# facebookresearch/DetectAndTrack

Measured on AMD Instinct MI355X. Metric: clips/sec (8-frame 800px), higher is better.
Workload: dtype bf16; 1 GPU; 3D R-18 FPN3D keypoint R-CNN inference, 4 clip(s) of 1x3x8x768x1344 per step (= per forward) per GPU (kT=3 body+FPN, slice-center 2D heads, per clip: 1000 proposals, 100 detections -> kps_score -> decoded keypoints); mode=infer, weights=random-init (synthetic_params, seed 3), images_per_forward=4, forwards_in_flight=3, clips_in_flight=12, keyframe_dce=False, hip_graph=True, resident_input=True, parallelism=clip-sharded x1 (no data-path collective)

## Files before the change

detectandtrack_amd/core/clip_graph.py:

```python
import numpy as np
import torch

from detectandtrack_amd import workspace as wsmod
from detectandtrack_amd.core import test as engine


def ops_ws_generation():
    from detectandtrack_amd.ops import hip_ops as ops
    return ops.ws_info()[2]


class ClipGraph(object):

    def __init__(self, model, ws, data_like, im_info, im_shape, stream=None, warmup=2, static_data=None, trunk=None):
        self.trunk = trunk
        assert engine.device_results_supported(), 'graph capture needs the device-side post-processing (cfg.HIP.DEVICE_BOX_RESULTS)'
        self.model, self.ws = model, ws
        B = int(trunk[3]) if trunk is not None else int(data_like.shape[0])
        self.scales = [float(v) for v in np.asarray(im_info, dtype=np.float64).reshape(-1, 3)[:, 2]]
        self.im_info = np.asarray(im_info, dtype=np.float32).reshape(-1, 3)
        assert self.im_info.shape[0] == B, 'im_info has %d rows for a blob of %d images' % (self.im_info.shape[0], B)
        self.im_shapes = [tuple(im_shape)] * B if not isinstance(im_shape[0], (tuple, list)) else [tuple(sh) for sh in im_shape]
        assert len(self.im_shapes) == B
        self.stream = stream or torch.cuda.current_stream()
# ... 7 lines not shown
        ws.FeedBlob('im_info', self.im_info)
        with torch.cuda.stream(self.stream):
            for _ in range(warmup):
                self._enqueue()
        torch.cuda.synchronize()
        self.graph = torch.cuda.CUDAGraph()
        with torch.cuda.graph(self.graph, stream=self.stream, capture_error_mode='thread_local'):
            self.dev = self._enqueue()
        torch.cuda.synchronize()
        self.blobs = dict(ws.blobs)
        with torch.cuda.stream(self.stream):
            self.ws_generation = ops_ws_generation()

    def _enqueue(self):
        prev, wsmod._GLOBAL = wsmod._GLOBAL, self.ws
        try:
            if self.trunk is not None:
                self.ws.trunk_ready = self.trunk
            else:
                self.ws.FeedBlob('data', self.static_data)
            self.ws.RunNet(self.model.net.name)
            return engine.enqueue_results_on_device(self.model, self.im_shapes, list(self.scales))
        finally:
            wsmod._GLOBAL = prev

    def launch(self, data_dev, im_info=None, im_shape=None):
        if self.trunk is not None:
            with torch.cuda.stream(self.stream):
                self.graph.replay()
            return self.dev
        assert tuple(data_dev.shape) == tuple(self.static_data.shape), \
            'graph captured for a %s blob, launched with %s' % (tuple(self.static_data.shape), tuple(data_dev.shape))
        if im_info is not None:
            assert np.array_equal(np.asarray(im_info, np.float32).reshape(-1, 3), self.im_info), \
                'graph captured for im_info %s, launched with %s' % (self.im_info.tolist(), np.asarray(im_info).tolist())
        if im_shape is not None:
            shapes = [tuple(im_shape)] * len(self.im_shapes) if not isinstance(im_shape[0], (tuple, list)) else [tuple(sh) for sh in im_shape]
            assert [sh[:2] for sh in shapes] == [sh[:2] for sh in self.im_shapes], (shapes, self.im_shapes)
        with torch.cuda.stream(self.stream):
# ... 17 lines not shown
```

detectandtrack_amd/core/config.py:

```python
import copy
import os
import os.path as osp
from ast import literal_eval

import numpy as np
import yaml

from detectandtrack_amd.utils.collections import AttrDict

_DEFAULTS_YAML = r"""
TRAIN:
  WEIGHTS: ''
  DATASET: ''
  SCALES: [600]
  MAX_SIZE: 1000
  IMS_PER_BATCH: 2
  BATCH_SIZE_PER_IM: 64
  FG_FRACTION: 0.25
  FG_THRESH: 0.5
  BG_THRESH_HI: 0.5
  BG_THRESH_LO: 0.0
  USE_FLIPPED: true
  BBOX_REG: true
  BBOX_THRESH: 0.5
# ... 187 lines not shown


def _to_attr(d, key=None):
    if isinstance(d, dict):
        return AttrDict({k: _to_attr(v, k) for k, v in d.items()})
    if isinstance(d, list) and key in _TUPLE_KEYS:
        return tuple(d)
    return d


def _build_defaults():
    c = _to_attr(yaml.safe_load(_DEFAULTS_YAML))
    c.BBOX_XFORM_CLIP = np.log(1000. / 16.)
    c.PIXEL_MEANS = np.array([[[102.9801, 115.9465, 122.7717]]])
    c.ROOT_DIR = os.getcwd()
    c.HIP = AttrDict({'DTYPE': 'bf16', 'KEYFRAME_DCE': False, 'DEVICE_KPS_DECODE': True, 'FRAME_TRUNK_CACHE': 0,
                      'DEVICE_BOX_RESULTS': True, 'FUSE_STEM_POOL': True, 'RCCL_DIRECT': False,
                      'PIPELINE_DEPTH': 4, 'CLIP_GRAPH': True, 'IMS_PER_FORWARD': 1, 'FUSE_RELU_BWD': True, 'FUSE_RELU_SUM_BWD': True, 'PERSISTENT_CU_SHARE': 50, 'DET_SPARE_ROWS': 4,
                      'DEFER_WGRAD_FINISH': True, 'MAX_GRAPHS_PER_SLOT': 6, 'PAD_TAIL_FORWARD': True,
                      'OVERLAP_ALLREDUCE': True, 'WGRAD_PW_BATCH': 16, 'DEVICE_ROI_SAMPLING': True, 'DECONV_GROUP_IGNORED': False, 'STEM_FROM_UINT8': True,
                      'TRAIN_GROUPED_CONV': False, 'USE_GN': False, 'GN_NUM_GROUPS': 32, 'GN_EPSILON': 1e-5, 'GN_KPS_HEAD': False,
                      'TUBE_SOFT_NMS': False, 'TRACK_CNN_WEIGHTS': '',
                      'TUBE_NMS_OKS': False, 'NMS_OKS_THRESH': 0.3,
                      'NONLOCAL': '', 'NONLOCAL_MAXPOOL': True, 'NONLOCAL_SCALE': True})
    return c


__C = _build_defaults()
cfg = __C
cfg_default = copy.deepcopy(__C)


def reset_cfg():
    fresh = copy.deepcopy(cfg_default)
    for k in list(__C.keys()):
        del __C[k]
    for k, v in fresh.items():
        __C[k] = v

# ... 91 lines not shown
```

detectandtrack_amd/core/pipeline.py:

```python
import collections
import os
import time

import numpy as np
import torch

from detectandtrack_amd.core.config import cfg
from detectandtrack_amd.core import test as engine
from detectandtrack_amd import workspace as wsmod


def _cu_masked_stream(spec):
    import ctypes
    bits = 0
    for part in spec.split('+'):
        lo, hi = [int(v) for v in part.split('-')]
        for b in range(lo, hi + 1):
            bits |= 1 << b
    words = (ctypes.c_uint32 * 8)(*[(bits >> (32 * i)) & 0xffffffff for i in range(8)])
    hip = ctypes.CDLL('libamdhip64.so')
    st = ctypes.c_void_p()
    rc = hip.hipExtStreamCreateWithCUMask(ctypes.byref(st), 8, words)
    assert rc == 0, 'hipExtStreamCreateWithCUMask failed: %d' % rc
    return torch.cuda.ExternalStream(st.value)
# ... 192 lines not shown
            g = s.graphs.get(key)
            if g is None:
                from detectandtrack_amd.core.clip_graph import ClipGraph
                while len(s.graphs) >= self.max_graphs:
                    _, old = s.graphs.popitem(last=False)
                    del old
                    self.graphs_evicted += 1
                g = s.graphs[key] = ClipGraph(self.model, s.ws, data_dev, im_info, im_shapes, stream=s.stream,
                                              static_data=data_dev if in_place else None, trunk=trunk)
                self.graphs_captured += 1
            else:
                s.graphs.move_to_end(key)
            return g.launch(data_dev, im_info=im_info, im_shape=im_shapes), g
        with torch.cuda.stream(s.stream):
            prev, wsmod._GLOBAL = wsmod._GLOBAL, s.ws
            try:
                if trunk is not None:
                    s.ws.trunk_ready = trunk
                else:
                    s.ws.FeedBlob('data', data_dev)
                s.ws.FeedBlob('im_info', np.asarray(im_info, np.float32))
                s.ws.RunNet(self.model.net.name)
                scales = [float(v) for v in np.asarray(im_info, np.float64).reshape(-1, 3)[:, 2]]
                return engine.enqueue_results_on_device(self.model, list(im_shapes), scales), None
            finally:
                wsmod._GLOBAL = prev

    def submit(self, data_dev, im_info, im_shape, tag=None, resident=False):
        slot = self._acquire()
        t0 = time.perf_counter()
        B = int(data_dev.shape[0])
        im_info = np.asarray(im_info, np.float64).reshape(-1, 3)
        assert im_info.shape[0] == B, (im_info.shape, B)
        shapes = [tuple(im_shape)] * B if not isinstance(im_shape[0], (tuple, list)) else [tuple(sh) for sh in im_shape]
        dev, g = self._enqueue(slot, data_dev, im_info, shapes, in_place=False, resident=resident and self.use_graph)
        self.slots[slot].event.record(self.slots[slot].stream)
        self.host_enqueue_s += time.perf_counter() - t0
        self.pending.append((slot, tag, im_info, shapes, dev, None, g))

    def _submit_frames_cached(self, clips, tag, frame_ids):
        from detectandtrack_amd.ops import hip_ops as ops
# ... 154 lines not shown
```

detectandtrack_amd/core/test.py:

```python
from collections import defaultdict

import numpy as np

from detectandtrack_amd.core.config import cfg
from detectandtrack_amd.core.nms_wrapper import nms, soft_nms
from detectandtrack_amd.ops.hip_ops import SOFT_NMS_MAX_BOXES
from detectandtrack_amd.ops.hip_ops import OKS_NMS_MAX_ROWS
from detectandtrack_amd.utils.timer import Timer
from detectandtrack_amd import workspace
import detectandtrack_amd.utils.blob as blob_utils
import detectandtrack_amd.utils.boxes as box_utils
import detectandtrack_amd.utils.keypoints as keypoint_utils


def _get_image_blob(im, num_frames=None):
    per_frame, scales = [], []
    for frame in im:
        ims, sc = blob_utils.prep_im_for_blob(frame, cfg.PIXEL_MEANS, cfg.TEST.SCALES, cfg.TEST.MAX_SIZE)
        per_frame.append(ims)
        scales.append(sc)
    for s in scales:
        assert scales[0] == s
    processed = [frames[i] for i in range(len(per_frame[0])) for frames in per_frame]
    return blob_utils.im_list_to_blob(processed, num_frames), np.array(scales[0])
# ... 169 lines not shown
def _nms_oks_on_device():
    return bool((not _tube_detections() or cfg.HIP.TUBE_NMS_OKS) and cfg.MODEL.NUM_CLASSES == 2 and cfg.KRCNN.NUM_KEYPOINTS == 17 and
                _device_out_cap() <= OKS_NMS_MAX_ROWS)


def device_results_supported():
    return bool(cfg.HIP.DEVICE_BOX_RESULTS and cfg.MODEL.FASTER_RCNN and cfg.TEST.BBOX_REG and
                not ((cfg.TEST.SOFT_NMS.ENABLED or cfg.TEST.BBOX_VOTE.ENABLED) and _tube_detections() and not cfg.HIP.TUBE_SOFT_NMS) and
                not (cfg.TEST.SOFT_NMS.ENABLED and cfg.TEST.RPN_POST_NMS_TOP_N > _soft_nms_capacity()) and
                not cfg.TEST.SVM and not (cfg.KRCNN.NMS_OKS and cfg.MODEL.KEYPOINTS_ON and not _nms_oks_on_device()) and
                (cfg.HIP.DEVICE_KPS_DECODE or not cfg.MODEL.KEYPOINTS_ON))


def rerun_rows_supported(need):
    return not (cfg.KRCNN.NMS_OKS and cfg.MODEL.KEYPOINTS_ON) or int(need) <= OKS_NMS_MAX_ROWS


def enqueue_results_on_device(model, im_shape, im_scale, out_cap=None, image=None):
    from detectandtrack_amd.ops import hip_ops as ops
    ws = workspace.GlobalWorkspace()
    rois = ws.blobs['rois']
    assert rois.kind == 'rois' and rois.count is not None, 'device post-processing expects the on-device proposal blob'
    ni = int(rois.count.numel())
    prob = workspace.blob_as_matrix(ws.blobs['cls_prob'])
    pred = workspace.blob_as_matrix(ws.blobs['bbox_pred'])
    rois_t, rois_n = rois.t if rois.t.dim() == 2 else rois.t.view(-1, rois.t.shape[-1]), rois.count
    if image is not None:
        seg = int(rois_t.shape[0]) // ni
        lo = int(image) * seg
        rois_t, rois_n = rois_t[lo:lo + seg], rois.count.view(-1)[int(image):int(image) + 1]
# ... 7 lines not shown
    dets, kp_rois, n_out = ops.box_results(
        rois_t, rois_n, prob, pred, cfg.MODEL.NUM_CLASSES, T, im_scale, im_shape, cfg.MODEL.BBOX_REG_WEIGHTS,
        float(np.float32(cfg.BBOX_XFORM_CLIP)), cfg.TEST.SCORE_THRESH, cfg.TEST.NMS, D, out_cap,
        cls_agnostic=cfg.MODEL.CLS_AGNOSTIC_BBOX_REG, n_images=ni,
        soft_nms=dict(method=cfg.TEST.SOFT_NMS.METHOD, sigma=cfg.TEST.SOFT_NMS.SIGMA, score_thresh=0.0001)
        if cfg.TEST.SOFT_NMS.ENABLED else None,
        bbox_vote=cfg.TEST.BBOX_VOTE.VOTE_TH if cfg.TEST.BBOX_VOTE.ENABLED else None,
        tubes=bool(cfg.HIP.TUBE_SOFT_NMS))
    xy = None
    if cfg.MODEL.KEYPOINTS_ON:
        if image is not None:
            kp_rois[:, 0] = float(image)
        b = workspace.Blob(kp_rois, 'mat')
        b.count = n_out[0:1] if ni == 1 else n_out[:, 0]
        ws.blobs['keypoint_rois'] = b
        workspace.RunNet(model.keypoint_net.Proto().name)
        heat = ws.blobs['kps_score'].t
        assert heat.shape[1] == cfg.KRCNN.NUM_KEYPOINTS * T, 'Heatmaps must be 17xT'
        xy = ops.heatmaps_to_keypoints(heat.contiguous(), dets, T, cfg.KRCNN.NUM_KEYPOINTS,
                                       cfg.KRCNN.INFERENCE_MIN_SIZE)
        if cfg.KRCNN.NMS_OKS:
            keypoint_utils.check_nms_oks_config()
            dets, xy, _, n_keep = ops.oks_nms(xy, dets, b.count, ni, T, cfg.KRCNN.NUM_KEYPOINTS, cfg.HIP.NMS_OKS_THRESH)
            return dets, n_out, xy, n_keep
    return dets, n_out, xy


def _split_results(d, keyps, num_classes):
    cls_boxes = [[] for _ in range(num_classes)]
    cls_keyps = [[] for _ in range(num_classes)] if keyps is not None else None
    for j in range(1, num_classes):
        sel = np.where(d[:, -1] == j)[0]
        cls_boxes[j] = d[sel, :-1]
        if keyps is not None and j == keypoint_utils.get_person_class_index():
            cls_keyps[j] = [keyps[i] for i in sel]
# ... 130 lines not shown
```

detectandtrack_amd/csrc/elementwise.hip:

```cpp
#include <algorithm>
#include <stdlib.h>

#include "dat_common.h"

namespace {

constexpr int TPB = 256;
inline int grid_for(size_t n, int per_thread = 1) {
    size_t b = (n + (size_t)TPB * per_thread - 1) / ((size_t)TPB * per_thread);
    const size_t cap = 256 * 16;
    return (int)(b < 1 ? 1 : (b > cap ? cap : b));
}

__global__ void zero_even_kernel(float* x, long long n) {
    const long long half = (n + 1) / 2;
    for (long long i = blockIdx.x * (long long)blockDim.x + threadIdx.x; i < half; i += (long long)gridDim.x * blockDim.x)
        x[2 * i] = 0.f;
}

template <bool HAS_BIAS>
__global__ void affine_nd_kernel(const float* __restrict__ x, const float* __restrict__ scale,
                                 const float* __restrict__ bias, float* __restrict__ y, int C, long long inner,
                                 long long total) {
    if ((inner & 3) == 0) {
// ... 177 lines not shown
                if (x >= L) continue;
                const int kx = ox + pad - up * x;
                const float fx = 1.f - fabsf((float)kx - center) / factor;
                const size_t fr = (size_t)r * Tr + t;
                const float v = ElemOf<DT>::ld(sub, ((fr * S + (y >> 1)) * S + (x >> 1)) * cs + ((y & 1) * 2 + (x & 1)) * K + k);
                acc += v * (fy * fx);
            }
        }
        out[i] = acc;
    }
}

template <int DT>
__global__ void kps_finalize_tile_kernel(const void* __restrict__ sub, int S, int cs, int K, int up, float* __restrict__ out) {
    extern __shared__ float low[];
    const int L = 2 * S, M = L * up;
    const int ksz = 2 * up, pad = up / 2;
    const float factor = (float)((ksz + 1) / 2);
    const float center = (ksz % 2 == 1) ? factor - 1.f : factor - 0.5f;
    const int fr = blockIdx.x / K, k = blockIdx.x - fr * K;
    for (int i = threadIdx.x; i < S * S * 4; i += blockDim.x) {
        const int cell = i >> 2, ab = i & 3;
        const int ys = cell / S, xs = cell - ys * S;
        low[(2 * ys + (ab >> 1)) * L + 2 * xs + (ab & 1)] = ElemOf<DT>::ld(sub, ((size_t)fr * S * S + cell) * cs + ab * K + k);
    }
    __syncthreads();
    const int ox = threadIdx.x % M, og = threadIdx.x / M, ng = blockDim.x / M;
    const int x_hi = (ox + pad) / up;
    float* const obase = out + (size_t)blockIdx.x * M * M;
    if (up == 2) {
        const int xa = x_hi, xb = x_hi - 1;
        const bool vxa = xa < L, vxb = xb >= 0;
        const float fxa = 1.f - fabsf((float)(ox + pad - up * xa) - center) / factor;
        const float fxb = 1.f - fabsf((float)(ox + pad - up * xb) - center) / factor;
        for (int oy = og; oy < M; oy += ng) {
            const int ya = (oy + pad) / up, yb = ya - 1;
            const float fya = 1.f - fabsf((float)(oy + pad - up * ya) - center) / factor;
            const float fyb = 1.f - fabsf((float)(oy + pad - up * yb) - center) / factor;
            float acc = 0.f;
            if (ya < L) {
                if (vxa) acc += low[ya * L + xa] * (fya * fxa);
                if (vxb) acc += low[ya * L + xb] * (fya * fxb);
            }
            if (yb >= 0) {
                if (vxa) acc += low[yb * L + xa] * (fyb * fxa);
                if (vxb) acc += low[yb * L + xb] * (fyb * fxb);
            }
            obase[(size_t)oy * M + ox] = acc;
        }
        return;
    }
    for (int oy = og; oy < M; oy += ng) {
        const int y_hi = (oy + pad) / up;
        float acc = 0.f;
        for (int y = y_hi; y >= 0 && oy + pad - up * y < ksz; --y) {
            if (y >= L) continue;
            const int ky = oy + pad - up * y;
            const float fy = 1.f - fabsf((float)ky - center) / factor;
            for (int x = x_hi; x >= 0 && ox + pad - up * x < ksz; --x) {
                if (x >= L) continue;
                const int kx = ox + pad - up * x;
                const float fx = 1.f - fabsf((float)kx - center) / factor;
                acc += low[y * L + x] * (fy * fx);
            }
        }
        obase[(size_t)oy * M + ox] = acc;
    }
}

}

#define DISPATCH_DT(dtype, KERNEL, grid, block, st, ...)                                                  \
    do {                                                                                                  \
        if ((dtype) == DAT_BF16)                                                                          \
            hipLaunchKernelGGL((KERNEL<DAT_BF16>), grid, block, 0, st, __VA_ARGS__);                      \
        else                                                                                              \
            hipLaunchKernelGGL((KERNEL<DAT_F32>), grid, block, 0, st, __VA_ARGS__);                       \
    } while (0)

__global__ void split_bf16x2_kernel(const float* __restrict__ x, uint4* __restrict__ y, long long n8, int c8) {
    for (long long i = blockIdx.x * (long long)blockDim.x + threadIdx.x; i < n8; i += (long long)gridDim.x * blockDim.x) {
        const long long pos = i / c8;
// ... 186 lines not shown
```

detectandtrack_amd/csrc/keypoints.hip:

```cpp
#include "dat_common.h"

namespace {

struct KpParams {
    const float* maps;
    const float* boxes;
    float* out;
    int R, T, K, M, min_size;
    int box_ld;
};

__device__ __forceinline__ void cubic(float t, float c[4]) {
    const float a = -0.75f;
    c[0] = ((a * (t + 1.f) - 5.f * a) * (t + 1.f) + 8.f * a) * (t + 1.f) - 4.f * a;
    c[1] = ((a + 2.f) * t - (a + 3.f)) * t * t + 1.f;
    c[2] = ((a + 2.f) * (1.f - t) - (a + 3.f)) * (1.f - t) * (1.f - t) + 1.f;
    c[3] = 1.0f - c[0] - c[1] - c[2];
}

__device__ __forceinline__ void resample(int src_len, int dst_len, int d, int& i0, float& frac) {
    const double step = 1.0 / ((double)dst_len / (double)src_len);
    const float f = (float)(((double)d + 0.5) * step - 0.5);
    const float fl = floorf(f);
    i0 = (int)fl;
// ... 66 lines not shown
        const int pos = red_i[0];
        const int x_int = pos % mw, y_int = (pos - x_int) / mw;
        const float w_corr = width / (float)mw, h_corr = height / (float)mh;
        const int TK = p.T * p.K, col = t * p.K + k;
        float* o = p.out + (size_t)r * 4 * TK;
        o[0 * TK + col] = (float)(((double)x_int + 0.5) * (double)w_corr + (double)off_x);
        o[1 * TK + col] = (float)(((double)y_int + 0.5) * (double)h_corr + (double)off_y);
        o[2 * TK + col] = red_v[0];
        o[3 * TK + col] = 1.f / red_s[0];
    }
}

constexpr int KD_STRIP = 64;
constexpr int KD_HP = KD_STRIP + 4;

__global__ __launch_bounds__(256) void kps_decode_sep_kernel(const KpParams p) {
    extern __shared__ __attribute__((aligned(16))) float smem_kd[];
    __shared__ float red_v[256];
    __shared__ int red_i[256];
    __shared__ float red_m[256], red_s[256];
    const int tid = threadIdx.x;
    const int k = blockIdx.x % p.K;
    const int t = (blockIdx.x / p.K) % p.T;
    const int r = blockIdx.x / (p.K * p.T);
    const int M = p.M;
    float* map = smem_kd;
    float* Hs = map + ((M * M + 3) & ~3);
    const float* src = p.maps + ((size_t)r * p.T * p.K + (size_t)t * p.K + k) * M * M;
    for (int i = tid; i < M * M; i += 256) map[i] = src[i];

    const float* b = p.boxes + (size_t)r * p.box_ld + t * 4;
    const float off_x = b[0], off_y = b[1];
    const float width = fmaxf(b[2] - b[0], 1.f), height = fmaxf(b[3] - b[1], 1.f);
    int mw = (int)ceilf(width), mh = (int)ceilf(height);
    if (p.min_size > 0) { mw = max(mw, p.min_size); mh = max(mh, p.min_size); }
    const double step_x = 1.0 / ((double)mw / (double)M), step_y = 1.0 / ((double)mh / (double)M);

    float best = -INFINITY;
    int best_i = 0x7fffffff;
    float run_m = -INFINITY, run_s = 0.f;
    const int hx = tid & 63, hr = tid >> 6;
    const int rl = tid >> 2, q = tid & 3;
    for (int x_base = 0; x_base < mw; x_base += KD_STRIP) {
        const int ncol = min(KD_STRIP, mw - x_base);
// ... 70 lines not shown
            red_m[tid] = mm; red_s[tid] = s;
        }
        __syncthreads();
    }
    if (tid == 0) {
        const int pos = red_i[0];
        const int x_int = pos % mw, y_int = (pos - x_int) / mw;
        const float w_corr = width / (float)mw, h_corr = height / (float)mh;
        const int TK = p.T * p.K, col = t * p.K + k;
        float* o = p.out + (size_t)r * 4 * TK;
        o[0 * TK + col] = (float)(((double)x_int + 0.5) * (double)w_corr + (double)off_x);
        o[1 * TK + col] = (float)(((double)y_int + 0.5) * (double)h_corr + (double)off_y);
        o[2 * TK + col] = red_v[0];
        o[3 * TK + col] = 1.f / red_s[0];
    }
}

}

extern "C" int dat_heatmaps_to_keypoints_ld(dat_ctx* ctx, dat_stream s, const float* maps, const float* boxes, int box_ld, int R, int T,
                                            int K, int M, int min_size, float* out);

extern "C" int dat_heatmaps_to_keypoints(dat_ctx* ctx, dat_stream s, const float* maps, const float* boxes, int R, int T,
                                         int K, int M, int min_size, float* out) {
    return dat_heatmaps_to_keypoints_ld(ctx, s, maps, boxes, 4 * T, R, T, K, M, min_size, out);
}

extern "C" int dat_heatmaps_to_keypoints_ld(dat_ctx* ctx, dat_stream s, const float* maps, const float* boxes, int box_ld, int R, int T,
                                            int K, int M, int min_size, float* out) {
    DAT_ENFORCE(ctx, maps && boxes && out && box_ld >= 4 * T, "heatmaps_to_keypoints: null argument / box row stride %d < 4 T", box_ld);
    DAT_ENFORCE(ctx, T >= 1 && K >= 1 && M >= 2 && (size_t)M * M * 4 <= 64 * 1024, "heatmaps_to_keypoints: T %d K %d M %d unsupported", T, K, M);
    if (R == 0) return DAT_OK;
    KpParams p;
    p.maps = maps; p.boxes = boxes; p.out = out; p.R = R; p.T = T; p.K = K; p.M = M; p.min_size = min_size; p.box_ld = box_ld;
    const size_t lds_sep = ((((size_t)M * M + 3) & ~(size_t)3) + (size_t)M * KD_HP) * 4;
    bool sep = ctx->dbg_kps_sep && lds_sep + 4096 <= 160 * 1024;
    if (sep && lds_sep + 4096 > 64 * 1024 && dat_ensure_lds(ctx, (const void*)kps_decode_sep_kernel, 160 * 1024) != DAT_OK) sep = false;
    if (sep) {
        hipLaunchKernelGGL(kps_decode_sep_kernel, dim3((unsigned)(R * T * K)), dim3(256), lds_sep, (hipStream_t)s, p);
    } else
        hipLaunchKernelGGL(kps_decode_kernel, dim3((unsigned)(R * T * K)), dim3(256), (size_t)M * M * 4, (hipStream_t)s, p);
    DAT_CHECK_LAUNCH(ctx, "heatmaps_to_keypoints");
    return DAT_OK;
}
```

detectandtrack_amd/libdat.py:

```python
import ctypes as C
import os

_HERE = os.path.dirname(os.path.abspath(__file__))
H16 = os.environ.get('DAT_H16', 'bf16')
assert H16 in ('bf16', 'fp16'), 'DAT_H16: bf16 | fp16'
LIB_PATH = os.environ.get('DAT_LIB', os.path.join(_HERE, 'libdat_hip_f16.so' if H16 == 'fp16' else 'libdat_hip.so'))

DAT_F32, DAT_BF16, DAT_BF16X3 = 0, 1, 2
DAT_OK = 0


class DatError(RuntimeError):
    """Raised for a non-zero C-ABI return code; message = dat_last_error() (the CAFFE_ENFORCE analogue)."""


class ConvDesc(C.Structure):
    _fields_ = [(n, C.c_int) for n in (
        'dtype', 'frames', 'T', 'H', 'W', 'Cin', 'Cout', 'out_cstride', 'KT', 'KH', 'KW',
        'stride_h', 'stride_w', 'pad_t', 'pad_h', 'pad_w', 'relu', 'res_mode', 'out_t0', 'out_tn', 'in_t0', 'in_tn', 'plan_frames', 'dil_h', 'dil_w')]


class PackItem(C.Structure):
    _fields_ = [('w', C.c_void_p), ('packed', C.c_void_p), ('scale', C.c_void_p)] + \
               [(n, C.c_int) for n in ('rows', 'cols', 'ntap', 'cout_pad', 'cin', 'dgrad', 'dtype', 'tile0', 'tiles_x', 'cit')]
# ... 116 lines not shown
    'dat_soft_nms_host': (_i, [C.POINTER(_f), _i, _f, _f, _f, _i, C.POINTER(_f), C.POINTER(_i), C.POINTER(_i)]),
    'dat_soft_nms_tubes_max_boxes': (_i, [_i]),
    'dat_soft_nms_tubes': (_i, [_p, _p, _p, _i, _i, _f, _f, _f, _i, _p, _p, _p]),
    'dat_soft_nms_tubes_host': (_i, [C.POINTER(_f), _i, _i, _f, _f, _f, _i, C.POINTER(_f), C.POINTER(_i), C.POINTER(_i)]),
    'dat_box_voting_tubes': (_i, [_p, _p, _p, _i, _p, _i, _i, _f, _p]),
    'dat_deconv_k4s2_weights': (_i, [_p, _p, _p, _i, _i, _p]),
    'dat_kps_finalize': (_i, [_p, _p, _i, _p, _i, _i, _i, _i, _i, _i, _p]),
    'dat_stem_conv_weight_bytes': (C.c_size_t, [_i]),
    'dat_stem_conv_pack_weights': (_i, [_p, _p, _i, _p, _i, _p]),
    'dat_stem_conv': (_i, [_p, _p, _i, _p, _p, _p, _p, _i, _i, _i, _i, _i, _p]),
    'dat_stem_conv_pool': (_i, [_p, _p, _i, _p, _p, _p, _p, _i, _i, _i, _i, _i, _p]),
    'dat_preprocess_frames': (_i, [_p, _p, _p, _i, _i, _i, _i, _d, _d, _i, _i, _i, _i, C.POINTER(_d), _p]),
    'dat_stem_conv_pool_u8': (_i, [_p, _p, _i, _p, _i, _i, _i, _d, _d, _i, _i, _i, _i, C.POINTER(_d), _p, _p, _p, _i, _p]),
    'dat_heatmaps_to_keypoints': (_i, [_p, _p, _p, _p, _i, _i, _i, _i, _i, _p]),
    'dat_heatmaps_to_keypoints_ld': (_i, [_p, _p, _p, _p, _i, _i, _i, _i, _i, _i, _p]),
    'dat_conv3d_wgrad_workspace_bytes': (C.c_size_t, [C.POINTER(ConvDesc), _i, _i]),
    'dat_conv3d_wgrad': (_i, [_p, _p, C.POINTER(ConvDesc), _p, _p, _i, _i, _i, _p, _p, _p]),
    'dat_conv3d_wgrad_acc_supported': (_i, [_p, C.POINTER(ConvDesc), _i]),
    'dat_conv3d_wgrad_acc': (_i, [_p, _p, C.POINTER(ConvDesc), _p, _p, _i, _i, _i, _p]),
    'dat_wgrad_finish_batch': (_i, [_p, _p, _p, _i, C.c_longlong]),
    'dat_conv3d_wgrad_acc_batch': (_i, [_p, _p, C.POINTER(WgradJob), _i]),
    'dat_relu_bias_bwd': (_i, [_p, _p, _i, _p, _p, _p, _p, _p, C.c_longlong, _i, _i, _i]),
    'dat_bn_workspace_bytes': (C.c_size_t, [_i, _ll, _i]),
    'dat_bn_stats': (_i, [_p, _p, _i, _p, _ll, _i, _i, _p, _p, _f, _f, _p, _p, _p, _p, _p, _p, _p, C.c_size_t]),
    'dat_bn_apply': (_i, [_p, _p, _i, _p, _p, _p, _p, _p, _ll, _i, _i, _i]),
    'dat_bn_bwd_reduce': (_i, [_p, _p, _i, _p, _p, _p, _p, _p, _p, _ll, _ll, _ll, _i, _i, _i, _p, _p, _p, _p, C.c_size_t]),
    'dat_bn_bwd_apply': (_i, [_p, _p, _i, _p, _p, _p, _p, _p, _p, _p, _ll, _ll, _ll, _i, _i]),
    'dat_gn_workspace_bytes': (C.c_size_t, [_i, _i, _ll, _i]),
    'dat_gn_stats': (_i, [_p, _p, _i, _p, _i, _ll, _i, _i, _i, _p, _p, _f, _p, _p, _p, _p, _p, C.c_size_t]),
    'dat_gn_apply': (_i, [_p, _p, _i, _p, _p, _p, _p, _p, _i, _ll, _i, _i, _i]),
# ... 66 lines not shown
```

detectandtrack_amd/ops/hip_ops.py:

```python
import ctypes as C

import numpy as np
import torch

from .. import libdat as L

F32, BF16 = L.DAT_F32, L.DAT_BF16


H16_DTYPE = torch.float16 if L.H16 == 'fp16' else torch.bfloat16


def tdtype(dt):
    return H16_DTYPE if dt == BF16 else torch.float32


def _ptr(t):
    return C.c_void_p(t.data_ptr()) if t is not None else None


_raw_stream = getattr(torch._C, '_cuda_getCurrentRawStream', None)


def _stream_handle(device=None):
# ... 1211 lines not shown
    if rc != L.DAT_OK:
        raise L.DatError('dat_oks_nms_host: bad arguments (%d)' % rc)
    keep = keep[:nk.value]
    return (keep, scores[:n], oks[:n, :n]) if want_oks else (keep, scores[:n])


def heatmaps_to_keypoints(maps, boxes, T, K, min_size=0):
    R, TK, M, M2 = maps.shape
    assert TK == T * K and M == M2 and boxes.dim() == 2 and boxes.shape[0] == R and boxes.shape[1] >= 4 * T
    assert maps.dtype == torch.float32 and boxes.dtype == torch.float32 and maps.is_contiguous() and boxes.is_contiguous()
    out = torch.empty((R, 4, TK), dtype=torch.float32, device=maps.device)
    ctx().call('dat_heatmaps_to_keypoints_ld', _stream(), _ptr(maps), _ptr(boxes), int(boxes.shape[1]), R, T, K, M, int(min_size), _ptr(out))
    return out


class ConvProfiler(object):

    def __init__(self, capacity=4096):
        self.capacity = capacity

    def start(self):
        L.lib().dat_prof_enable(ctx().h, self.capacity)

    def stop(self):
        tags = (C.c_int * self.capacity)()
        flops = (C.c_double * self.capacity)()
        ms = (C.c_float * self.capacity)()
        n = L.lib().dat_prof_read(ctx().h, self.capacity, tags, flops, ms)
        mhz = C.c_double(0.0)
        L.lib().dat_prof_clock(ctx().h, C.byref(mhz))
# ... 4 lines not shown
```

detectandtrack_amd/workspace.py:

```python
import collections
import logging

import numpy as np
import torch

from detectandtrack_amd.core.config import cfg
from detectandtrack_amd.ops import hip_ops as ops

logger = logging.getLogger(__name__)


class Blob(object):
    __slots__ = ('t', 'kind', 'N', 'T', 'C', 'dt', 'five_d', 'count', 'sigmoid_of', 'host', 'keyframe', 't2c', 'split', 'tsel', 'bn', 'roi')

    def __init__(self, t, kind, N=1, T=1, C=0, dt=0, five_d=False, count=None):
        self.t, self.kind, self.N, self.T, self.C, self.dt = t, kind, N, T, C, dt
        self.five_d = five_d
        self.count = count
        self.roi = False
        self.sigmoid_of = None
        self.host = None
        self.split = None
        self.tsel = None
        self.t2c = False
        self.keyframe = None
        self.bn = None


class Workspace(object):
    def __init__(self, device=0, dtype=None):
        self.device = torch.device('cuda', device)
        self.dtype = dtype
        self.blobs = {}
        self.params = {}
        self.nets = {}
        self._layers = {}
        self._dev_params = {}
        self.conv_log = None
        self.train_sampler = None
        self.trunk_cache = collections.OrderedDict()
        self.trunk_request = None
        self.trunk_ready = None

    def FeedBlob(self, name, arr):
# ... 39 lines not shown
    def HasBlob(self, name):
        return _unscoped(name) in self.blobs or _unscoped(name) in self.params

    def Blobs(self):
        return list(self.blobs.keys())

    _READER_KEYS = ('slice_lazy', 'pad_unread', 'conv_reader')

    def CreateNet(self, net):
        check_bn_sees_every_frame(net)
        self.nets[net.name] = net
        for k in [k for k in self._layers if isinstance(k, tuple) and k and k[0] in self._READER_KEYS]:
            del self._layers[k]
        return net

    def RunNet(self, name):
        name = getattr(name, 'name', name)
        net = self.nets[name]
        Executor(self, net).run()

    def ResetWorkspace(self):
        self.blobs.clear()
        self._layers.clear()
        self._dev_params.clear()
        self.trunk_cache.clear()
        self.trunk_request = None

    def trunk_missing(self, frame_ids):
        seen, out = set(), []
        for fid in frame_ids:
            if fid not in self.trunk_cache and fid not in seen:
                seen.add(fid)
                out.append(fid)
        return out
# ... 119 lines not shown
    return w if w.dim() == 5 else w.unsqueeze(2)


class Executor(object):

    _PAD_BLIND = frozenset(['Softmax', 'Sigmoid', 'BilinearInterpolation', 'GenerateProposals', 'TimeMean', 'RpnDeltasPerFrame'])
    training = False
    _TSEL_AWARE = frozenset(['Conv', 'RoIFeatureTransform'])

    def __init__(self, ws, net):
        check_bn_sees_every_frame(net)
        self.ws, self.net = ws, net
        self.pending_rpn = []
        self.has_collect = any(op.type == 'CollectAndDistributeFpnRpnProposals' for op in net.ops)

    def run(self):
        self._plan_rpn_siblings()
        self._plan_keyframe_dce()
        start = self._run_cached_trunk()
        ready = getattr(self.ws, 'trunk_ready', None)
        if ready is not None:
            self.ws.trunk_ready = None
            start, live, t, N, T, C, dt = ready
            self.ws.blobs[live] = Blob(t, 'fmap', N, T, C, dt, True)
        blobs = self.ws.blobs
        for i, op in enumerate(self.net.ops):
            if i < start or i in self._skip:
                continue
            if op.type not in self._TSEL_AWARE:
                for n in op.inputs:
                    b = blobs.get(n)
                    assert b is None or b.tsel is None, 'op %d (%s) reads the lazily sliced blob %r' % (i, op.type, n)
            getattr(self, 'op_' + op.type)(i, op)

    @staticmethod
    def trunk_split(net):
        n_max, produced = 0, []
        have = set()
        for op in net.ops:
            a = op.args if isinstance(op.args, dict) else {}
            ok = (op.type == 'Conv' and a.get('kernels', [2])[0] == 1 and op.inputs[0] in have | {'data'} and
                  (not a.get('residual') or a['residual'] in have) and not a.get('res_mode') == 2) or \
                 (op.type in ('MaxPool', 'StopGradient') and op.inputs[0] in have)
# ... 694 lines not shown
    GlobalWorkspace().FeedBlob(name, arr)


def FetchBlob(name):
    return GlobalWorkspace().FetchBlob(name)


def HasBlob(name):
    return GlobalWorkspace().HasBlob(name)


def CreateNet(net):
    return GlobalWorkspace().CreateNet(net)


def RunNet(name):
    GlobalWorkspace().RunNet(name)
```

include/dat_hip.h:

```cpp
#ifndef DAT_HIP_H_
#define DAT_HIP_H_

#include <stddef.h>
#include <stdint.h>

#ifdef __cplusplus
extern "C" {
#endif

typedef struct dat_ctx dat_ctx;
typedef void* dat_stream;

enum { DAT_F32 = 0, DAT_BF16 = 1,
       DAT_BF16X3 = 2 };
enum { DAT_OK = 0, DAT_ERR_ARG = -1, DAT_ERR_LAUNCH = -2, DAT_ERR_ALLOC = -3, DAT_ERR_UNSUPPORTED = -4 };

int dat_version(void);
int dat_h16_format(void);
int dat_ctx_create(dat_ctx** out, int device);
void dat_ctx_destroy(dat_ctx* ctx);
const char* dat_last_error(dat_ctx* ctx);
int dat_ws_info(dat_ctx* ctx, void** ptr, size_t* bytes, int* generation);
int dat_ws_reserve(dat_ctx* ctx, size_t bytes);
int dat_fill_zero(dat_ctx* ctx, dat_stream s, void* ptr, size_t bytes);
// ... 198 lines not shown
                       const float* bias, int relu, int N, int T, int H, int W, void* out_pool);
int dat_stem_conv_pool_u8(dat_ctx* ctx, dat_stream s, int dtype, const unsigned char* frames, int n_frames, int h, int w, double fx, double fy,
                          int out_h, int out_w, int pad_h, int pad_w, const double* pixel_means, const void* w_packed, const float* scale,
                          const float* bias, int relu, void* out_pool);

typedef struct dat_comm dat_comm;
int dat_comm_unique_id(dat_ctx* ctx, void* id128);
int dat_comm_init_rank(dat_ctx* ctx, const void* id128, int nranks, int rank, dat_comm** out);
int dat_allreduce_bucket(dat_ctx* ctx, dat_stream s, dat_comm* comm, float* buf, size_t count);
int dat_comm_destroy(dat_comm* comm);

int dat_heatmaps_to_keypoints(dat_ctx* ctx, dat_stream s, const float* maps, const float* boxes, int R, int T, int K,
                              int M, int min_size, float* out);
int dat_heatmaps_to_keypoints_ld(dat_ctx* ctx, dat_stream s, const float* maps, const float* boxes, int box_ld, int R, int T, int K, int M,
                                 int min_size, float* out);

size_t dat_conv3d_wgrad_workspace_bytes(const dat_conv_desc* d, int Cin_real, int Cout_real);
int dat_conv3d_wgrad(dat_ctx* ctx, dat_stream s, const dat_conv_desc* d, const void* x, const void* g, int g_cstride,
                     int Cin_real, int Cout_real, const float* scale, void* workspace, float* dW);
typedef struct dat_wfinish_item {
    const float* Gt;
    const float* scale;
    float* dW;
    int Cout, Cin, ntaps, accumulate;
    long long block0;
} dat_wfinish_item;
int dat_conv3d_wgrad_acc_supported(dat_ctx* ctx, const dat_conv_desc* d, int g_cstride);
int dat_conv3d_wgrad_acc(dat_ctx* ctx, dat_stream s, const dat_conv_desc* d, const void* x, const void* g, int g_cstride,
                         int Cin_real, int Cout_real, float* Gt);
int dat_wgrad_finish_batch(dat_ctx* ctx, dat_stream s, const dat_wfinish_item* items_dev, int n, long long total_blocks);
// ... 105 lines not shown
```

Before: 265.5 clips/s.

## Fuse keypoint heatmap upsampling into the device keypoint decode kernel

When the keypoint net ends in a BilinearInterpolation producing kps_score and the heatmap fits in LDS, the net now stops before that op. A new fused kernel unfolds the low-res sub-pixel map, upsamples it into shared memory and runs the separable argmax decode in one launch. This avoids writing the full-resolution 17-channel heatmaps to global memory and reading them back, and drops one launch per step. The cost is a new code path gated by a workspace flag and a map-size limit, with more LDS per block and possibly lower occupancy.

```diff
diff --git a/detectandtrack_amd/core/clip_graph.py b/detectandtrack_amd/core/clip_graph.py
--- a/detectandtrack_amd/core/clip_graph.py
+++ b/detectandtrack_amd/core/clip_graph.py
@@ -45,6 +45,7 @@
 
     def _enqueue(self):
         prev, wsmod._GLOBAL = wsmod._GLOBAL, self.ws
+        self.ws.kps_score_unread = True
         try:
             if self.trunk is not None:
                 self.ws.trunk_ready = self.trunk
@@ -54,6 +55,7 @@
             return engine.enqueue_results_on_device(self.model, self.im_shapes, list(self.scales))
         finally:
             wsmod._GLOBAL = prev
+            self.ws.kps_score_unread = False
 
     def launch(self, data_dev, im_info=None, im_shape=None):
         if self.trunk is not None:
diff --git a/detectandtrack_amd/core/config.py b/detectandtrack_amd/core/config.py
--- a/detectandtrack_amd/core/config.py
+++ b/detectandtrack_amd/core/config.py
@@ -225,7 +225,7 @@
     c.BBOX_XFORM_CLIP = np.log(1000. / 16.)
     c.PIXEL_MEANS = np.array([[[102.9801, 115.9465, 122.7717]]])
     c.ROOT_DIR = os.getcwd()
-    c.HIP = AttrDict({'DTYPE': 'bf16', 'KEYFRAME_DCE': False, 'DEVICE_KPS_DECODE': True, 'FRAME_TRUNK_CACHE': 0,
+    c.HIP =AttrDict({'DTYPE': 'bf16', 'KEYFRAME_DCE': False, 'DEVICE_KPS_DECODE': True, 'FRAME_TRUNK_CACHE': 0,
                       'DEVICE_BOX_RESULTS': True, 'FUSE_STEM_POOL': True, 'RCCL_DIRECT': False,
                       'PIPELINE_DEPTH': 4, 'CLIP_GRAPH': True, 'IMS_PER_FORWARD': 1, 'FUSE_RELU_BWD': True, 'FUSE_RELU_SUM_BWD': True, 'PERSISTENT_CU_SHARE': 50, 'DET_SPARE_ROWS': 4,
                       'DEFER_WGRAD_FINISH': True, 'MAX_GRAPHS_PER_SLOT': 6, 'PAD_TAIL_FORWARD': True,
@@ -233,7 +233,7 @@
                       'TRAIN_GROUPED_CONV': False, 'USE_GN': False, 'GN_NUM_GROUPS': 32, 'GN_EPSILON': 1e-5, 'GN_KPS_HEAD': False,
                       'TUBE_SOFT_NMS': False, 'TRACK_CNN_WEIGHTS': '',
                       'TUBE_NMS_OKS': False, 'NMS_OKS_THRESH': 0.3,
-                      'NONLOCAL': '', 'NONLOCAL_MAXPOOL': True, 'NONLOCAL_SCALE': True})
+                      'NONLOCAL': '', 'NONLOCAL_MAXPOOL': True, 'NONLOCAL_SCALE': True, 'FUSE_KPS_DECODE': True})
     return c
 
 
diff --git a/detectandtrack_amd/core/pipeline.py b/detectandtrack_amd/core/pipeline.py
--- a/detectandtrack_amd/core/pipeline.py
+++ b/detectandtrack_amd/core/pipeline.py
@@ -230,6 +230,7 @@
             return g.launch(data_dev, im_info=im_info, im_shape=im_shapes), g
         with torch.cuda.stream(s.stream):
             prev, wsmod._GLOBAL = wsmod._GLOBAL, s.ws
+            s.ws.kps_score_unread = True
             try:
                 if trunk is not None:
                     s.ws.trunk_ready = trunk
@@ -241,6 +242,7 @@
                 return engine.enqueue_results_on_device(self.model, list(im_shapes), scales), None
             finally:
                 wsmod._GLOBAL = prev
+                s.ws.kps_score_unread = False
 
     def submit(self, data_dev, im_info, im_shape, tag=None, resident=False):
         slot = self._acquire()
diff --git a/detectandtrack_amd/core/test.py b/detectandtrack_amd/core/test.py
--- a/detectandtrack_amd/core/test.py
+++ b/detectandtrack_amd/core/test.py
@@ -207,6 +207,17 @@
 
 def rerun_rows_supported(need):
     return not (cfg.KRCNN.NMS_OKS and cfg.MODEL.KEYPOINTS_ON) or int(need) <= OKS_NMS_MAX_ROWS
+
+
+def _fusable_kps_tail(ws, model, T):
+    from detectandtrack_amd.ops.hip_ops import KPS_FUSED_MAX_M
+    if not cfg.HIP.get('FUSE_KPS_DECODE', True) or T != 1 or cfg.KRCNN.HEATMAP_SIZE > KPS_FUSED_MAX_M:
+        return None
+    net_ops = ws.nets[model.keypoint_net.Proto().name].ops
+    last = net_ops[-1]
+    if last.type != 'BilinearInterpolation' or list(last.outputs) != ['kps_score']:
+        return None
+    return len(net_ops) - 1
 
 
 def enqueue_results_on_device(model, im_shape, im_scale, out_cap=None, image=None):
@@ -244,11 +255,20 @@
         b = workspace.Blob(kp_rois, 'mat')
         b.count = n_out[0:1] if ni == 1 else n_out[:, 0]
         ws.blobs['keypoint_rois'] = b
-        workspace.RunNet(model.keypoint_net.Proto().name)
-        heat = ws.blobs['kps_score'].t
-        assert heat.shape[1] == cfg.KRCNN.NUM_KEYPOINTS * T, 'Heatmaps must be 17xT'
-        xy = ops.heatmaps_to_keypoints(heat.contiguous(), dets, T, cfg.KRCNN.NUM_KEYPOINTS,
-                                       cfg.KRCNN.INFERENCE_MIN_SIZE)
+        tail = _fusable_kps_tail(ws, model, T) if ws.kps_score_unread else None
+        if tail is not None:
+            workspace.RunNet(model.keypoint_net.Proto().name, stop_before=tail)
+            op = ws.nets[model.keypoint_net.Proto().name].ops[tail]
+            ws.blobs.pop(op.outputs[0], None)
+            x = ws.blobs[op.inputs[0]]
+            assert x.T == 1 and op.args['dim'] == cfg.KRCNN.NUM_KEYPOINTS and x.N == dets.shape[0], (x.T, op.args['dim'], x.N, dets.shape)
+            xy = ops.kps_decode_fused(x.t, x.dt, x.N, 1, cfg.KRCNN.NUM_KEYPOINTS, op.args['up_scale'], dets, cfg.KRCNN.INFERENCE_MIN_SIZE)
+        else:
+            workspace.RunNet(model.keypoint_net.Proto().name)
+            heat = ws.blobs['kps_score'].t
+            assert heat.shape[1] == cfg.KRCNN.NUM_KEYPOINTS * T, 'Heatmaps must be 17xT'
+            xy = ops.heatmaps_to_keypoints(heat.contiguous(), dets, T, cfg.KRCNN.NUM_KEYPOINTS,
+                                           cfg.KRCNN.INFERENCE_MIN_SIZE)
         if cfg.KRCNN.NMS_OKS:
             keypoint_utils.check_nms_oks_config()
             dets, xy, _, n_keep = ops.oks_nms(xy, dets, b.count, ni, T, cfg.KRCNN.NUM_KEYPOINTS, cfg.HIP.NMS_OKS_THRESH)
diff --git a/detectandtrack_amd/csrc/elementwise.hip b/detectandtrack_amd/csrc/elementwise.hip
--- a/detectandtrack_amd/csrc/elementwise.hip
+++ b/detectandtrack_amd/csrc/elementwise.hip
@@ -2,6 +2,7 @@
 #include <stdlib.h>
 
 #include "dat_common.h"
+#include "kps_tile.h"
 
 namespace {
 
@@ -215,58 +216,11 @@
 template <int DT>
 __global__ void kps_finalize_tile_kernel(const void* __restrict__ sub, int S, int cs, int K, int up, float* __restrict__ out) {
     extern __shared__ float low[];
-    const int L = 2 * S, M = L * up;
-    const int ksz = 2 * up, pad = up / 2;
-    const float factor = (float)((ksz + 1) / 2);
-    const float center = (ksz % 2 == 1) ? factor - 1.f : factor - 0.5f;
+    const int M = 2 * S * up;
     const int fr = blockIdx.x / K, k = blockIdx.x - fr * K;
-    for (int i = threadIdx.x; i < S * S * 4; i += blockDim.x) {
-        const int cell = i >> 2, ab = i & 3;
-        const int ys = cell / S, xs = cell - ys * S;
-        low[(2 * ys + (ab >> 1)) * L + 2 * xs + (ab & 1)] = ElemOf<DT>::ld(sub, ((size_t)fr * S * S + cell) * cs + ab * K + k);
-    }
+    kps_unfold_low<DT>(sub, fr, k, S, cs, K, low, threadIdx.x, blockDim.x);
     __syncthreads();
-    const int ox = threadIdx.x % M, og = threadIdx.x / M, ng = blockDim.x / M;
-    const int x_hi = (ox + pad) / up;
-    float* const obase = out + (size_t)blockIdx.x * M * M;
-    if (up == 2) {
-        const int xa = x_hi, xb = x_hi - 1;
-        const bool vxa = xa < L, vxb = xb >= 0;
-        const float fxa = 1.f - fabsf((float)(ox + pad - up * xa) - center) / factor;
-        const float fxb = 1.f - fabsf((float)(ox + pad - up * xb) - center) / factor;
-        for (int oy = og; oy < M; oy += ng) {
-            const int ya = (oy + pad) / up, yb = ya - 1;
-            const float fya = 1.f - fabsf((float)(oy + pad - up * ya) - center) / factor;
-            const float fyb = 1.f - fabsf((float)(oy + pad - up * yb) - center) / factor;
-            float acc = 0.f;
-            if (ya < L) {
-                if (vxa) acc += low[ya * L + xa] * (fya * fxa);
-                if (vxb) acc += low[ya * L + xb] * (fya * fxb);
-            }
-            if (yb >= 0) {
-                if (vxa) acc += low[yb * L + xa] * (fyb * fxa);
-                if (vxb) acc += low[yb * L + xb] * (fyb * fxb);
-            }
-            obase[(size_t)oy * M + ox] = acc;
-        }
-        return;
-    }
-    for (int oy = og; oy < M; oy += ng) {
-        const int y_hi = (oy + pad) / up;
-        float acc = 0.f;
-        for (int y = y_hi; y >= 0 && oy + pad - up * y < ksz; --y) {
-            if (y >= L) continue;
-            const int ky = oy + pad - up * y;
-            const float fy = 1.f - fabsf((float)ky - center) / factor;
-            for (int x = x_hi; x >= 0 && ox + pad - up * x < ksz; --x) {
-                if (x >= L) continue;
-                const int kx = ox + pad - up * x;
-                const float fx = 1.f - fabsf((float)kx - center) / factor;
-                acc += low[y * L + x] * (fy * fx);
-            }
-        }
-        obase[(size_t)oy * M + ox] = acc;
-    }
+    kps_upsample_map(low, S, up, out + (size_t)blockIdx.x * M * M, threadIdx.x, blockDim.x / M);
 }
 
 }
diff --git a/detectandtrack_amd/csrc/keypoints.hip b/detectandtrack_amd/csrc/keypoints.hip
--- a/detectandtrack_amd/csrc/keypoints.hip
+++ b/detectandtrack_amd/csrc/keypoints.hip
@@ -1,4 +1,5 @@
 #include "dat_common.h"
+#include "kps_tile.h"
 
 namespace {
 
@@ -104,8 +105,7 @@
 constexpr int KD_STRIP = 64;
 constexpr int KD_HP = KD_STRIP + 4;
 
-__global__ __launch_bounds__(256) void kps_decode_sep_kernel(const KpParams p) {
-    extern __shared__ __attribute__((aligned(16))) float smem_kd[];
+__device__ __forceinline__ void kps_decode_sep_map(const KpParams& p, const float* map, float* Hs) {
     __shared__ float red_v[256];
     __shared__ int red_i[256];
     __shared__ float red_m[256], red_s[256];
@@ -114,10 +114,6 @@
     const int t = (blockIdx.x / p.K) % p.T;
     const int r = blockIdx.x / (p.K * p.T);
     const int M = p.M;
-    float* map = smem_kd;
-    float* Hs = map + ((M * M + 3) & ~3);
-    const float* src = p.maps + ((size_t)r * p.T * p.K + (size_t)t * p.K + k) * M * M;
-    for (int i = tid; i < M * M; i += 256) map[i] = src[i];
 
     const float* b = p.boxes + (size_t)r * p.box_ld + t * 4;
     const float off_x = b[0], off_y = b[1];
@@ -218,6 +214,29 @@
         o[2 * TK + col] = red_v[0];
         o[3 * TK + col] = 1.f / red_s[0];
     }
+}
+
+__global__ __launch_bounds__(256) void kps_decode_sep_kernel(const KpParams p) {
+    extern __shared__ __attribute__((aligned(16))) float smem_kd[];
+    const int M = p.M;
+    float* map = smem_kd;
+    const float* src = p.maps + (size_t)blockIdx.x * M * M;
+    for (int i = threadIdx.x; i < M * M; i += 256) map[i] = src[i];
+    kps_decode_sep_map(p, map, map + ((M * M + 3) & ~3));
+}
+
+template <int DT>
+__global__ __launch_bounds__(256) void kps_decode_fused_kernel(const KpParams p, const void* __restrict__ sub, int S, int cs, int up) {
+    extern __shared__ __attribute__((aligned(16))) float smem_kd[];
+    const int M = p.M;
+    float* map = smem_kd;
+    float* Hs = map + ((M * M + 3) & ~3);
+    const int fr = blockIdx.x / p.K, k = blockIdx.x - fr * p.K;
+    kps_unfold_low<DT>(sub, fr, k, S, cs, p.K, Hs, threadIdx.x, 256);
+    __syncthreads();
+    const int ng = max(1, min(4, 256 / M));
+    if ((int)threadIdx.x < ng * M) kps_upsample_map(Hs, S, up, map, threadIdx.x, ng);
+    kps_decode_sep_map(p, map, Hs);
 }
 
 }
@@ -247,3 +266,26 @@
     DAT_CHECK_LAUNCH(ctx, "heatmaps_to_keypoints");
     return DAT_OK;
 }
+
+extern "C" int dat_kps_decode_fused(dat_ctx* ctx, dat_stream s, int dtype, const void* sub, int R, int Tr, int S, int cs, int K, int up,
+                                    const float* boxes, int box_ld, int min_size, float* out) {
+    DAT_ENFORCE(ctx, up >= 2 && up % 2 == 0, "kps_decode_fused: up_scale must be even (detector.py:354), got %d", up);
+    DAT_ENFORCE(ctx, K > 0 && 4 * K <= cs, "kps_decode_fused: the 4*K = %d sub-pixel channels do not fit the channel stride %d", 4 * K, cs);
+    DAT_ENFORCE(ctx, Tr >= 1 && S >= 1 && box_ld >= 4 * Tr, "kps_decode_fused: Tr %d S %d / box row stride %d < 4 Tr", Tr, S, box_ld);
+    const int M = 2 * S * up;
+    DAT_ENFORCE(ctx, M <= DAT_KPS_FUSED_MAX_M, "kps_decode_fused: maps of %d x %d exceed %d: run dat_kps_finalize and dat_heatmaps_to_keypoints", M, M,
+                DAT_KPS_FUSED_MAX_M);
+    DAT_ENFORCE(ctx, (long long)R * Tr * K < (1ll << 31), "kps_decode_fused: %lld maps", (long long)R * Tr * K);
+    if (R == 0) return DAT_OK;
+    DAT_ENFORCE(ctx, sub && boxes && out, "kps_decode_fused: null argument");
+    KpParams p;
+    p.maps = nullptr; p.boxes = boxes; p.out = out; p.R = R; p.T = Tr; p.K = K; p.M = M; p.min_size = min_size; p.box_ld = box_ld;
+    const size_t lds = ((((size_t)M * M + 3) & ~(size_t)3) + (size_t)M * KD_HP) * 4;
+    static_assert((DAT_KPS_FUSED_MAX_M * DAT_KPS_FUSED_MAX_M + DAT_KPS_FUSED_MAX_M * KD_HP) * 4 + 4096 <= 64 * 1024, "DAT_KPS_FUSED_MAX_M");
+    if (dtype == DAT_BF16)
+        hipLaunchKernelGGL((kps_decode_fused_kernel<DAT_BF16>), dim3((unsigned)(R * Tr * K)), dim3(256), lds, (hipStream_t)s, p, sub, S, cs, up);
+    else
+        hipLaunchKernelGGL((kps_decode_fused_kernel<DAT_F32>), dim3((unsigned)(R * Tr * K)), dim3(256), lds, (hipStream_t)s, p, sub, S, cs, up);
+    DAT_CHECK_LAUNCH(ctx, "kps_decode_fused");
+    return DAT_OK;
+}
diff --git a/detectandtrack_amd/csrc/kps_tile.h b/detectandtrack_amd/csrc/kps_tile.h
--- /dev/null
+++ b/detectandtrack_amd/csrc/kps_tile.h
@@ -0,0 +1,60 @@
+#pragma once
+#include "dat_common.h"
+
+template <int DT>
+__device__ __forceinline__ void kps_unfold_low(const void* __restrict__ sub, int fr, int k, int S, int cs, int K, float* low, int tid,
+                                               int nthr) {
+    const int L = 2 * S;
+    for (int i = tid; i < S * S * 4; i += nthr) {
+        const int cell = i >> 2, ab = i & 3;
+        const int ys = cell / S, xs = cell - ys * S;
+        low[(2 * ys + (ab >> 1)) * L + 2 * xs + (ab & 1)] = ElemOf<DT>::ld(sub, ((size_t)fr * S * S + cell) * cs + ab * K + k);
+    }
+}
+
+__device__ __forceinline__ void kps_upsample_map(const float* low, int S, int up, float* obase, int tid, int ng) {
+    const int L = 2 * S, M = L * up;
+    const int ksz = 2 * up, pad = up / 2;
+    const float factor = (float)((ksz + 1) / 2);
+    const float center = (ksz % 2 == 1) ? factor - 1.f : factor - 0.5f;
+    const int ox = tid % M, og = tid / M;
+    const int x_hi = (ox + pad) / up;
+    if (up == 2) {
+        const int xa = x_hi, xb = x_hi - 1;
+        const bool vxa = xa < L, vxb = xb >= 0;
+        const float fxa = 1.f - fabsf((float)(ox + pad - up * xa) - center) / factor;
+        const float fxb = 1.f - fabsf((float)(ox + pad - up * xb) - center) / factor;
+        for (int oy = og; oy < M; oy += ng) {
+            const int ya = (oy + pad) / up, yb = ya - 1;
+            const float fya = 1.f - fabsf((float)(oy + pad - up * ya) - center) / factor;
+            const float fyb = 1.f - fabsf((float)(oy + pad - up * yb) - center) / factor;
+            float acc = 0.f;
+            if (ya < L) {
+                if (vxa) acc = __builtin_fmaf(low[ya * L + xa], fya * fxa, acc);
+                if (vxb) acc = __builtin_fmaf(low[ya * L + xb], fya * fxb, acc);
+            }
+            if (yb >= 0) {
+                if (vxa) acc = __builtin_fmaf(low[yb * L + xa], fyb * fxa, acc);
+                if (vxb) acc = __builtin_fmaf(low[yb * L + xb], fyb * fxb, acc);
+            }
+            obase[(size_t)oy * M + ox] = acc;
+        }
+        return;
+    }
+    for (int oy = og; oy < M; oy += ng) {
+        const int y_hi = (oy + pad) / up;
+        float acc = 0.f;
+        for (int y = y_hi; y >= 0 && oy + pad - up * y < ksz; --y) {
+            if (y >= L) continue;
+            const int ky = oy + pad - up * y;
+            const float fy = 1.f - fabsf((float)ky - center) / factor;
+            for (int x = x_hi; x >= 0 && ox + pad - up * x < ksz; --x) {
+                if (x >= L) continue;
+                const int kx = ox + pad - up * x;
+                const float fx = 1.f - fabsf((float)kx - center) / factor;
+                acc = __builtin_fmaf(low[y * L + x], fy * fx, acc);
+            }
+        }
+        obase[(size_t)oy * M + ox] = acc;
+    }
+}
diff --git a/detectandtrack_amd/libdat.py b/detectandtrack_amd/libdat.py
--- a/detectandtrack_amd/libdat.py
+++ b/detectandtrack_amd/libdat.py
@@ -154,6 +154,7 @@
     'dat_stem_conv_pool_u8': (_i, [_p, _p, _i, _p, _i, _i, _i, _d, _d, _i, _i, _i, _i, C.POINTER(_d), _p, _p, _p, _i, _p]),
     'dat_heatmaps_to_keypoints': (_i, [_p, _p, _p, _p, _i, _i, _i, _i, _i, _p]),
     'dat_heatmaps_to_keypoints_ld': (_i, [_p, _p, _p, _p, _i, _i, _i, _i, _i, _i, _p]),
+    'dat_kps_decode_fused': (_i, [_p, _p, _i, _p, _i, _i, _i, _i, _i, _i, _p, _i, _i, _p]),
     'dat_conv3d_wgrad_workspace_bytes': (C.c_size_t, [C.POINTER(ConvDesc), _i, _i]),
     'dat_conv3d_wgrad': (_i, [_p, _p, C.POINTER(ConvDesc), _p, _p, _i, _i, _i, _p, _p, _p]),
     'dat_conv3d_wgrad_acc_supported': (_i, [_p, C.POINTER(ConvDesc), _i]),
diff --git a/detectandtrack_amd/ops/hip_ops.py b/detectandtrack_amd/ops/hip_ops.py
--- a/detectandtrack_amd/ops/hip_ops.py
+++ b/detectandtrack_amd/ops/hip_ops.py
@@ -1249,6 +1249,19 @@
     return out
 
 
+KPS_FUSED_MAX_M = 88
+
+
+def kps_decode_fused(sub, dtype, R, Tr, K, up, boxes, min_size=0):
+    f, s, s2, cs = sub.shape
+    assert f == R * Tr and s == s2 and 2 * s * up <= KPS_FUSED_MAX_M
+    assert boxes.dim() == 2 and boxes.shape[0] == R and boxes.shape[1] >= 4 * Tr and boxes.dtype == torch.float32 and boxes.is_contiguous()
+    out = torch.empty((R, 4, Tr * K), dtype=torch.float32, device=sub.device)
+    ctx().call('dat_kps_decode_fused', _stream(), dtype, _ptr(sub), R, Tr, s, cs, K, up, _ptr(boxes), int(boxes.shape[1]), int(min_size),
+               _ptr(out))
+    return out
+
+
 class ConvProfiler(object):
 
     def __init__(self, capacity=4096):
diff --git a/detectandtrack_amd/workspace.py b/detectandtrack_amd/workspace.py
--- a/detectandtrack_amd/workspace.py
+++ b/detectandtrack_amd/workspace.py
@@ -28,6 +28,8 @@
 
 
 class Workspace(object):
+    kps_score_unread = False
+
     def __init__(self, device=0, dtype=None):
         self.device = torch.device('cuda', device)
         self.dtype = dtype
@@ -97,10 +99,10 @@
             del self._layers[k]
         return net
 
-    def RunNet(self, name):
+    def RunNet(self, name, stop_before=None):
         name = getattr(name, 'name', name)
         net = self.nets[name]
-        Executor(self, net).run()
+        Executor(self, net).run(stop_before)
 
     def ResetWorkspace(self):
         self.blobs.clear()
@@ -250,7 +252,7 @@
         self.pending_rpn = []
         self.has_collect = any(op.type == 'CollectAndDistributeFpnRpnProposals' for op in net.ops)
 
-    def run(self):
+    def run(self, stop_before=None):
         self._plan_rpn_siblings()
         self._plan_keyframe_dce()
         start = self._run_cached_trunk()
@@ -263,6 +265,8 @@
         for i, op in enumerate(self.net.ops):
             if i < start or i in self._skip:
                 continue
+            if stop_before is not None and i >= stop_before:
+                break
             if op.type not in self._TSEL_AWARE:
                 for n in op.inputs:
                     b = blobs.get(n)
@@ -987,5 +991,5 @@
     return GlobalWorkspace().CreateNet(net)
 
 
-def RunNet(name):
-    GlobalWorkspace().RunNet(name)
+def RunNet(name, stop_before=None):
+    GlobalWorkspace().RunNet(name, stop_before)
diff --git a/include/dat_hip.h b/include/dat_hip.h
--- a/include/dat_hip.h
+++ b/include/dat_hip.h
@@ -236,6 +236,9 @@
                               int M, int min_size, float* out);
 int dat_heatmaps_to_keypoints_ld(dat_ctx* ctx, dat_stream s, const float* maps, const float* boxes, int box_ld, int R, int T, int K, int M,
                                  int min_size, float* out);
+#define DAT_KPS_FUSED_MAX_M 88
+int dat_kps_decode_fused(dat_ctx* ctx, dat_stream s, int dtype, const void* sub, int R, int Tr, int S, int cs, int K, int up,
+                         const float* boxes, int box_ld, int min_size, float* out);
 
 size_t dat_conv3d_wgrad_workspace_bytes(const dat_conv_desc* d, int Cin_real, int Cout_real);
 int dat_conv3d_wgrad(dat_ctx* ctx, dat_stream s, const dat_conv_desc* d, const void* x, const void* g, int g_cstride,
```

Measured after the change: 264.6 clips/s (median of 2 runs). About the same (-0.4%).
